# DylanAuty/ObjCAViT

Measured on AMD Instinct MI355X. Metric: images/sec (640x480, bs=16) forward depth inference, 3 batches of 16 in flight per GPU; AbsRel vs CPU ref, higher is better.
Workload: dtype f32 (fp16 / bf16 split contractions)

## Files before the change

include/objcavit_hip.h:

```cpp
#ifndef OBJCAVIT_HIP_H
#define OBJCAVIT_HIP_H

#include <stddef.h>
#include <stdint.h>

#ifdef __cplusplus
extern "C" {
#endif

typedef void* ocv_stream_t;

#define OCV_ABI_VERSION 5
int ocv_abi_version(void);
const char* ocv_last_error(void);

int ocv_range_flag_set(unsigned* flag);
int ocv_range_flag_take_fwd(unsigned* flag, unsigned* out, ocv_stream_t stream);
int ocv_attention_set_fp32_range(int on);
int ocv_attention_set_dispatch(int form);

#define OCV_ACT_NONE 0
#define OCV_ACT_RELU 1
#define OCV_ACT_LEAKY_RELU 2
#define OCV_ACT_SILU 3
// ... 164 lines not shown

int ocv_se_gate_fwd(const float* mean, const float* w1, const float* b1, const float* w2t, const float* b2, float* gate,
                    float* hidden_ws, int B, int C, int R, ocv_stream_t stream);

int ocv_conv_nhwc_fwd(const float* x1, int C1, const float* x2, int C2, const void* w_hi, const void* w_lo,
                      const float* bias, const float* residual, float* y, int B, int H, int W, int Cout, int ksize,
                      int act, ocv_stream_t stream);
int ocv_conv_nhwc_exact_fwd(const float* x1, int C1, const float* x2, int C2, const float* w_tap_major, const float* bias,
                            const float* residual, float* y, int B, int H, int W, int Cout, int ksize, int act,
                            ocv_stream_t stream);
int ocv_conv3x3_nhwc_strided_fwd(const float* x, int Cin, const void* w_hi, const void* w_lo, const float* bias,
                                 const float* residual, float* y, int B, int H, int W, int Cout, int stride, int pad_t,
                                 int pad_l, int Ho, int Wo, int act, ocv_stream_t stream);

int ocv_mbconv_expand_dw_tiles(int Ho, int Wo, int k, int stride);
int ocv_mbconv_expand_dw_fwd(const float* x, const void* w_packed, const float* bias_expand, const float* w_dw,
                             const float* bias_dw, float* y, float* part, int B, int H, int W, int Cin, int mid, int k,
                             int stride, int pad_t, int pad_l, int Ho, int Wo, ocv_stream_t stream);

size_t ocv_split_act_elems(int B, int H, int W, int C);

int ocv_conv_nhwc_split_fwd(const void* x_hl, int Cin, const void* w_hi, const void* w_lo, const float* bias,
                            const float* residual, float* y, void* y_hl, int B, int H, int W, int Cout, int ksize,
                            int act, ocv_stream_t stream);
size_t ocv_conv_nhwc_split_workspace_bytes(int B, int H, int W, int Cin, int Cout, int ksize);
int ocv_conv_nhwc_split_ws_fwd(const void* x_hl, int Cin, const void* w_hi, const void* w_lo, const float* bias,
                               const float* residual, float* y, void* y_hl, int B, int H, int W, int Cout, int ksize,
                               int act, void* workspace, size_t workspace_bytes, ocv_stream_t stream);
int ocv_conv_nhwc_split_x_fwd(const void* x_hl, int Cin, const void* w_hi, const void* w_lo, const float* oscale, int f16,
                              const float* bias, const float* residual, float* y, void* y_hl, int B, int H, int W, int Cout,
                              int ksize, int act, void* workspace, size_t workspace_bytes, ocv_stream_t stream);

int ocv_conv3x3_packed_taps_k(int Cin);
int ocv_conv3x3_split_packed_taps_fwd(const void* x_hl, int Cin, const void* w_hi, const void* w_lo, const float* oscale, int f16,
                                      const float* bias, const float* residual, float* y, void* y_hl, int B, int H, int W, int Cout,
                                      int act, ocv_stream_t stream);

size_t ocv_conv3x3_winograd43_workspace_bytes(int B, int H, int W, int Cin, int Cout);
int ocv_conv3x3_winograd43_split_fwd(const void* x_hl, int Cin, const void* u_hi, const void* u_lo, const float* fscale,
                                     const float* cscale, const float* bias, float* y, void* y_hl, int B, int H, int W, int Cout,
                                     int act, int hl_f16, void* workspace, size_t workspace_bytes, ocv_stream_t stream);

int ocv_tap_interp_supported(int h, int w, int H, int W, int Cout);
int ocv_tap_interp_staging_rounds(int h, int w, int H, int W);
int ocv_tap_interp_combine_fwd(const float* z, int h, int w, int zpad, const float* zborder, const float* s, const float* bias,
                               float* y, void* y_hl, int B, int H, int W, int Cout, int act, ocv_stream_t stream);
int ocv_tap_interp_combine_x_fwd(const float* z, int h, int w, int zpad, const float* zborder, const float* s, const float* bias,
                                 float* y, void* y_hl, int hl_f16, int B, int H, int W, int Cout, int act, ocv_stream_t stream);


int ocv_upsample_concat_split_fwd(const float* x, int h, int w, int C1, const float* skip, int C2, void* out_hl, int B,
                                  int H, int W, ocv_stream_t stream);
int ocv_upsample_concat_split_x_fwd(const float* x, int h, int w, int C1, const float* skip, int C2, void* out_hl, int f16, int B,
                                    int H, int W, ocv_stream_t stream);

size_t ocv_depth_metrics_workspace_bytes(int B, int H, int W);
int ocv_depth_metrics_fwd(const float* pred, const float* pred_mirror, int h, int w, const float* gt, int H, int W,
                          float min_depth, float max_depth, int crop_y0, int crop_y1, int crop_x0, int crop_x1,
                          long first_image_id, float* records, int B, void* workspace, size_t workspace_bytes,
                          ocv_stream_t stream);
size_t ocv_depth_metrics_loss_workspace_bytes(int B, int H, int W, int n_bins);
int ocv_depth_metrics_loss_fwd(const float* pred, const float* pred_mirror, int h, int w, const float* gt, int H, int W,
                               float min_depth, float max_depth, int crop_y0, int crop_y1, int crop_x0, int crop_x1,
                               const float* bin_edges, int n_bins, long first_image_id, float* records, float* loss_records, int B,
                               void* workspace, size_t workspace_bytes, ocv_stream_t stream);

// ... 53 lines not shown
```

objcavit_amd/_lib.py:

```python
from __future__ import annotations

import ctypes as C
import os
from typing import Optional

_HERE = os.path.dirname(os.path.abspath(__file__))
LIB_PATH = os.environ.get("OCV_LIB_PATH") or os.path.join(_HERE, "lib", "libobjcavit_hip.so")

_f32p = C.c_void_p
_u8p = C.c_void_p
_stream = C.c_void_p
ABI_VERSION = 5


class EncoderLayerParams(C.Structure):
    _fields_ = [("struct_size", C.c_size_t)] + [(n, C.c_void_p) for n in (
        "in_proj_w", "in_proj_b", "out_proj_w", "out_proj_b", "norm1_w", "norm1_b",
        "linear1_w", "linear1_b", "linear2_w", "linear2_b", "norm2_w", "norm2_b",
        "in_proj_p3", "out_proj_p3", "linear1_p3", "linear2_p3",
        "in_proj_h2", "out_proj_h2", "linear1_h2", "linear2_h2")]

    def __init__(self, *a, **kw):
        super().__init__(*a, **kw)
        self.struct_size = C.sizeof(EncoderLayerParams)
# ... 106 lines not shown
                                [C.c_int, _f32p, C.c_void_p, C.c_void_p, C.c_void_p, C.c_void_p, C.c_size_t, _stream]),
    "ocv_conv3x3_few_channels_fwd": (C.c_int, [_f32p, C.c_long, C.c_long, C.c_long, C.c_long, _f32p, _f32p] + [C.c_int] * 5 + [_stream]),
    "ocv_stem_conv_fwd": (C.c_int, [_f32p, _f32p, _f32p, _f32p] + [C.c_int] * 12 + [_stream]),
    "ocv_pointwise_packed_weight_elems": (C.c_size_t, [C.c_int, C.c_int]),
    "ocv_pointwise_split_set_dispatch": (C.c_int, [C.c_int, C.c_int, C.c_int]),
    "ocv_pointwise_conv_nhwc_split_fwd": (C.c_int, [_f32p, _f32p, C.c_int, C.c_void_p, _f32p, _f32p, _f32p,
                                                    C.c_long, C.c_int, C.c_int, C.c_int, C.c_void_p]),
    "ocv_pointwise_conv_nhwc_fwd": (C.c_int, [_f32p, _f32p, C.c_int, _f32p, _f32p, _f32p, _f32p, C.c_long, C.c_int, C.c_int,
                                              C.c_int, _stream]),
    "ocv_depthwise_conv_nhwc_fwd": (C.c_int, [_f32p, _f32p, _f32p, _f32p] + [C.c_int] * 11 + [_stream]),
    "ocv_channel_mean_workspace_bytes": (C.c_size_t, [C.c_int, C.c_int, C.c_long]),
    "ocv_channel_mean_nhwc_fwd": (C.c_int, [_f32p, _f32p, C.c_int, C.c_int, C.c_long, C.c_void_p, C.c_size_t, _stream]),
    "ocv_se_gate_fwd": (C.c_int, [_f32p] * 7 + [C.c_int] * 3 + [_stream]),
    "ocv_conv_nhwc_fwd": (C.c_int, [_f32p, C.c_int, _f32p, C.c_int, C.c_void_p, C.c_void_p, _f32p, _f32p, _f32p] +
                          [C.c_int] * 6 + [_stream]),
    "ocv_conv3x3_nhwc_strided_fwd": (C.c_int, [_f32p, C.c_int, C.c_void_p, C.c_void_p, _f32p, _f32p, _f32p] + [C.c_int] * 10 + [_stream]),
    "ocv_conv_nhwc_exact_fwd": (C.c_int, [_f32p, C.c_int, _f32p, C.c_int, _f32p, _f32p, _f32p, _f32p] + [C.c_int] * 6 + [_stream]),
    "ocv_mbconv_expand_dw_tiles": (C.c_int, [C.c_int] * 4),
    "ocv_mbconv_expand_dw_fwd": (C.c_int, [_f32p, C.c_void_p, _f32p, _f32p, _f32p, _f32p, _f32p] + [C.c_int] * 11 + [_stream]),
    "ocv_regressor_bins_fwd": (C.c_int, [_f32p, C.c_long, _f32p, _f32p, _f32p, _f32p, _f32p, _f32p, C.c_int, C.c_int, C.c_int, C.c_int, C.c_float,
                                         C.c_int, C.c_float, C.c_float, _f32p, _f32p, _f32p, C.c_int, _stream]),
    "ocv_bin_edges_fwd": (C.c_int, [_f32p, C.c_int, C.c_float, C.c_float, _f32p, _f32p, _f32p, C.c_int, C.c_int, _stream]),
    "ocv_object_tokens_pad_fwd": (C.c_int, [_f32p, C.c_void_p, C.c_float, _f32p, _u8p, C.c_int, C.c_int, C.c_int, _stream]),
    "ocv_object_front_pad_fwd": (C.c_int, [_f32p, C.c_void_p, C.c_int, C.c_int, C.c_float, _f32p, _u8p] + [C.c_int] * 4 + [_stream]),
    "ocv_split_act_elems": (C.c_size_t, [C.c_int] * 4),
    "ocv_conv_nhwc_split_fwd": (C.c_int, [C.c_void_p, C.c_int, C.c_void_p, C.c_void_p, _f32p, _f32p, _f32p, C.c_void_p]
                                + [C.c_int] * 6 + [_stream]),
    "ocv_conv_nhwc_split_workspace_bytes": (C.c_size_t, [C.c_int] * 6),
    "ocv_conv_nhwc_split_ws_fwd": (C.c_int, [C.c_void_p, C.c_int, C.c_void_p, C.c_void_p, _f32p, _f32p, _f32p, C.c_void_p]
                                   + [C.c_int] * 6 + [C.c_void_p, C.c_size_t, _stream]),
    "ocv_conv_nhwc_split_x_fwd": (C.c_int, [C.c_void_p, C.c_int, C.c_void_p, C.c_void_p, _f32p, C.c_int, _f32p, _f32p, _f32p, C.c_void_p]
                                  + [C.c_int] * 6 + [C.c_void_p, C.c_size_t, _stream]),
    "ocv_conv3x3_packed_taps_k": (C.c_int, [C.c_int]),
    "ocv_conv3x3_split_packed_taps_fwd": (C.c_int, [C.c_void_p, C.c_int, C.c_void_p, C.c_void_p, _f32p, C.c_int, _f32p, _f32p, _f32p, C.c_void_p]
                                          + [C.c_int] * 5 + [_stream]),
    "ocv_upsample_concat_split_x_fwd": (C.c_int, [_f32p, C.c_int, C.c_int, C.c_int, _f32p, C.c_int, C.c_void_p, C.c_int,
                                                  C.c_int, C.c_int, C.c_int, _stream]),
    "ocv_tap_interp_combine_x_fwd": (C.c_int, [_f32p, C.c_int, C.c_int, C.c_int, _f32p, _f32p, _f32p, _f32p, C.c_void_p] + [C.c_int] * 6 + [_stream]),
    "ocv_pos_grid_sample_fwd": (C.c_int, [_f32p, C.c_int, C.c_int, C.c_int, _f32p, C.c_int, C.c_int, C.c_int, C.c_float, C.c_float,
                                          C.c_int, _f32p, _f32p, _stream]),
    "ocv_conv3x3_winograd43_workspace_bytes": (C.c_size_t, [C.c_int] * 5),
    "ocv_conv3x3_winograd43_split_fwd": (C.c_int, [C.c_void_p, C.c_int, C.c_void_p, C.c_void_p, _f32p, _f32p, _f32p, _f32p, C.c_void_p] + [C.c_int] * 6 +
                                         [C.c_void_p, C.c_size_t, _stream]),
    "ocv_tap_interp_supported": (C.c_int, [C.c_int] * 5),
    "ocv_tap_interp_staging_rounds": (C.c_int, [C.c_int] * 4),
    "ocv_tap_interp_combine_fwd": (C.c_int, [_f32p, C.c_int, C.c_int, C.c_int, _f32p, _f32p, _f32p, _f32p, C.c_void_p] + [C.c_int] * 5 + [_stream]),
    "ocv_upsample_concat_split_fwd": (C.c_int, [_f32p, C.c_int, C.c_int, C.c_int, _f32p, C.c_int, C.c_void_p,
                                                C.c_int, C.c_int, C.c_int, _stream]),
}

_lib: Optional[C.CDLL] = None


class HipLibraryError(RuntimeError):
    pass


def load(path: Optional[str] = None) -> C.CDLL:
    global _lib
    if _lib is not None and path is None:
        return _lib
    import torch
    p = path or LIB_PATH
    if not os.path.exists(p):
        raise HipLibraryError(
            f"{p} not found: build it with `python -m objcavit_amd.build` (hipcc --offload-arch=gfx950). "
# ... 24 lines not shown
```

objcavit_amd/csrc/conv_igemm.hip:

```cpp
#include <stdlib.h>

#include "common.hpp"
#include "../../include/objcavit_hip.h"

namespace {

typedef __bf16 bf16x8 __attribute__((ext_vector_type(8)));
typedef _Float16 cv_h16x8 __attribute__((ext_vector_type(8)));
typedef _Float16 cv_h16x4 __attribute__((ext_vector_type(4)));
typedef __bf16 ti4 __attribute__((ext_vector_type(4)));

constexpr int CBM = 256, CBN = 128, CBK = 32;
constexpr int ROWB = 80;
constexpr int A_BYTES = CBM * ROWB, B_BYTES = CBN * ROWB;
constexpr int BUF_BYTES = 2 * A_BYTES + 2 * B_BYTES;

struct ConvArgs {
  const float* x1; const float* x2;
  const __bf16* xhl;
  __bf16* yhl;
  int Cpo;
  const __bf16* whi; const __bf16* wlo;
  const float* bias; const float* res; float* y;
  int C1, C2, Cin, Cp, Cout, H, W, ks, act;
  int Ho, Wo, pad_t, pad_l;
  long M;
  int mtiles, ntiles;
  int ksplit;
  int zbatch;
  long xz_bytes, wz_bytes;
  int zflat;
  int f16;
  const float* oscale;
  unsigned* range_flag;
  unsigned rowpitch;
  int gpt, gpt_inv;
  int Kp;
};

__device__ __forceinline__ f32x4 gload16(const void* p) { return *reinterpret_cast<const f32x4*>(p); }

__device__ __forceinline__ void split4(const f32x4 v, __bf16* hi, __bf16* lo) {
  const float f[4] = {v[0], v[1], v[2], v[3]};
#pragma unroll
  for (int i = 0; i < 4; ++i) {
    const __bf16 h = (__bf16)f[i];
    hi[i] = h;
    lo[i] = (__bf16)(f[i] - (float)h);
  }
}

__device__ __forceinline__ void split4h(const f32x4 v, _Float16* hi, _Float16* lo) {
  const float f[4] = {v[0], v[1], v[2], v[3]};
#pragma unroll
  for (int i = 0; i < 4; ++i) {
    const _Float16 h = (_Float16)f[i];
    hi[i] = h;
    lo[i] = (_Float16)(f[i] - (float)h);
  }
}
template <bool F16>
__device__ __forceinline__ void split4_bits(const f32x4 v, unsigned short* hi, unsigned short* lo) {
  if constexpr (F16) split4h(v, reinterpret_cast<_Float16*>(hi), reinterpret_cast<_Float16*>(lo));
  else split4(v, reinterpret_cast<__bf16*>(hi), reinterpret_cast<__bf16*>(lo));
}
__device__ __forceinline__ void split4_bits(const f32x4 v, unsigned short* hi, unsigned short* lo, bool f16) {
  if (f16) split4_bits<true>(v, hi, lo);
  else split4_bits<false>(v, hi, lo);
}
__device__ __forceinline__ f32x4 join4_bits(const void* p, int lo_off, bool f16) {
// ... 200 lines not shown
  __syncthreads();
  for (int t = 0; t < nsteps; ++t) {
    if ((t & 1) == g) {
      if (t + 2 < nsteps) convert(raw, cvt);
      __syncthreads();
    } else {
      if (t + 1 >= 2 && t + 1 < nsteps) write_lds((t + 1) & 1, raw, cvt);
      if (t + 3 < nsteps) issue_loads(raw);
      __syncthreads();
    }
  }
}

}


namespace {

typedef __attribute__((address_space(1))) const void* gptr_t;
typedef __attribute__((address_space(3))) void* lptr_t;

constexpr int DROW = 64;
constexpr int DA = CBM * DROW, DB = CBN * DROW;
constexpr int DBUF = 2 * DA + 2 * DB;
constexpr int DNBUF = 3;

constexpr int ERS = 68;
__device__ __forceinline__ float conv_act(float v, int act) {
  if (act == OCV_ACT_LEAKY_RELU) return v > 0.f ? v : 0.01f * v;
  if (act == OCV_ACT_SILU) return fast_silu(v);
  if (act == OCV_ACT_RELU) return fmaxf(v, 0.f);
  return v;
}
template <bool F16>
__device__ __forceinline__ void conv_store_rows(const ConvArgs& p, const unsigned char* lds, int wave, int lane, long m0, int n0,
                                                long yoff) {
  const int cw = wave & 3, half = wave >> 2;
  const int wm = cw >> 1, wn = cw & 1;
  const float* tile = reinterpret_cast<const float*>(lds) + cw * (128 * ERS);
  const int oct = lane & 7, rsub = lane >> 3;
  const int ncol = n0 + wn * 64 + oct * 8;
  if (ncol >= p.Cout) return;
  float bv[8], sv[8];
#pragma unroll
  for (int e = 0; e < 8; ++e) {
    bv[e] = p.bias != nullptr ? p.bias[ncol + e] : 0.f;
    sv[e] = p.oscale != nullptr ? p.oscale[ncol + e] : 1.f;
  }
  float amax = 0.f;
#pragma unroll 4
  for (int it = 0; it < 8; ++it) {
    const int row = half * 64 + it * 8 + rsub;
    const long m = m0 + wm * 128 + row;
    if (m >= p.M) continue;
    f32x4 a = *reinterpret_cast<const f32x4*>(tile + row * ERS + oct * 8);
    f32x4 c = *reinterpret_cast<const f32x4*>(tile + row * ERS + oct * 8 + 4);
#pragma unroll
    for (int e = 0; e < 4; ++e) {
      a[e] = conv_act(fmaf(a[e], sv[e], bv[e]), p.act);
      c[e] = conv_act(fmaf(c[e], sv[4 + e], bv[4 + e]), p.act);
    }
    const long o = m * p.Cout + ncol;
    if (p.res != nullptr) {
      a += *reinterpret_cast<const f32x4*>(p.res + o);
      c += *reinterpret_cast<const f32x4*>(p.res + o + 4);
    }
    if (p.y != nullptr) {
      *reinterpret_cast<f32x4*>(p.y + yoff + o) = a;
      *reinterpret_cast<f32x4*>(p.y + yoff + o + 4) = c;
    }
    if (p.yhl != nullptr) {
      __attribute__((aligned(16))) unsigned short hi[8], lo[8];
      split4_bits<F16>(a, hi, lo);
      split4_bits<F16>(c, hi + 4, lo + 4);
      if constexpr (F16) amax = ocv_amax4(ocv_amax4(amax, a), c);
      const long oh = hl_index(m, ncol, p.Cpo);
      *reinterpret_cast<bf16x8*>(p.yhl + oh) = *reinterpret_cast<bf16x8*>(hi);
      *reinterpret_cast<bf16x8*>(p.yhl + oh + 32) = *reinterpret_cast<bf16x8*>(lo);
    }
  }
  if constexpr (F16) ocv_range_note(p.range_flag, amax);
}

template <bool F16>
__global__ __launch_bounds__(512) void conv_split_dma_kernel(ConvArgs p) {
  extern __shared__ __attribute__((aligned(1024))) unsigned char lds[];
// ... 54 lines not shown
        bl[j] = *reinterpret_cast<const bf16x8*>(pb + DB + j * 16 * DROW);
      }
#pragma unroll
      for (int i = 0; i < 8; ++i) {
        ah[i] = *reinterpret_cast<const bf16x8*>(pa + i * 16 * DROW);
        al[i] = *reinterpret_cast<const bf16x8*>(pa + DA + i * 16 * DROW);
      }
#pragma unroll
      for (int i = 0; i < 8; ++i)
#pragma unroll
        for (int j = 0; j < 4; ++j) {
          if constexpr (F16) {
            acc[i][j] = __builtin_amdgcn_mfma_f32_16x16x32_f16(__builtin_bit_cast(cv_h16x8, ah[i]), __builtin_bit_cast(cv_h16x8, bh[j]), acc[i][j], 0, 0, 0);
            acc[i][j] = __builtin_amdgcn_mfma_f32_16x16x32_f16(__builtin_bit_cast(cv_h16x8, ah[i]), __builtin_bit_cast(cv_h16x8, bl[j]), acc[i][j], 0, 0, 0);
            acc[i][j] = __builtin_amdgcn_mfma_f32_16x16x32_f16(__builtin_bit_cast(cv_h16x8, al[i]), __builtin_bit_cast(cv_h16x8, bh[j]), acc[i][j], 0, 0, 0);
          } else {
            acc[i][j] = __builtin_amdgcn_mfma_f32_16x16x32_bf16(ah[i], bh[j], acc[i][j], 0, 0, 0);
            acc[i][j] = __builtin_amdgcn_mfma_f32_16x16x32_bf16(ah[i], bl[j], acc[i][j], 0, 0, 0);
            acc[i][j] = __builtin_amdgcn_mfma_f32_16x16x32_bf16(al[i], bh[j], acc[i][j], 0, 0, 0);
          }
        }
      __syncthreads();
    }

    if ((p.Cout & 7) == 0) {
      float* tile = reinterpret_cast<float*>(lds) + wave * (128 * ERS);
#pragma unroll
      for (int j = 0; j < 4; ++j)
#pragma unroll
        for (int i = 0; i < 8; ++i)
#pragma unroll
          for (int r = 0; r < 4; ++r) tile[(16 * i + 4 * q4 + r) * ERS + 16 * j + l15] = acc[i][j][r];
      __syncthreads();
      conv_store_rows<F16>(p, lds, wave, lane, m0, n0, yoff);
      return;
    }
#pragma unroll
    for (int j = 0; j < 4; ++j) {
      const int n = n0 + wn * 64 + j * 16 + l15;
      const bool nok = n < p.Cout;
      const float bv = (p.bias != nullptr && nok) ? p.bias[n] : 0.f;
      const float sv = (p.oscale != nullptr && nok) ? p.oscale[n] : 1.f;
#pragma unroll
      for (int i = 0; i < 8; ++i)
#pragma unroll
        for (int r = 0; r < 4; ++r) {
          const long m = m0 + wm * 128 + i * 16 + 4 * q4 + r;
          if (nok && m < p.M) {
            float v = fmaf(acc[i][j][r], sv, bv);
            if (p.act == OCV_ACT_LEAKY_RELU) v = v > 0.f ? v : 0.01f * v;
            else if (p.act == OCV_ACT_SILU) v = fast_silu(v);
            else if (p.act == OCV_ACT_RELU) v = fmaxf(v, 0.f);
            if (p.res != nullptr) v += p.res[m * p.Cout + n];
            if (p.y != nullptr) p.y[yoff + m * p.Cout + n] = v;
            if (p.yhl != nullptr) {
              if constexpr (F16) {
                ocv_range_note(p.range_flag, fabsf(v));
                _Float16* yh = reinterpret_cast<_Float16*>(p.yhl);
                const _Float16 hb = (_Float16)v;
                yh[hl_index(m, n, p.Cpo)] = hb;
                yh[hl_index(m, n, p.Cpo) + 32] = (_Float16)(v - (float)hb);
              } else {
                const __bf16 hb = (__bf16)v;
                p.yhl[hl_index(m, n, p.Cpo)] = hb;
                p.yhl[hl_index(m, n, p.Cpo) + 32] = (__bf16)(v - (float)hb);
              }
            }
// ... 94 lines not shown
    for (int i = 0; i < 2; ++i) {
      unsigned char* dst = base + 2 * DA + (32 * pw + 16 * i) * DROW;
      __builtin_amdgcn_global_load_lds((gptr_t)(whz_ + woff + rbB[i]), (lptr_t)dst, 16, 0, 0);
      __builtin_amdgcn_global_load_lds((gptr_t)(wlz_ + woff + rbB[i]), (lptr_t)(dst + DB), 16, 0, 0);
    }
  };

  auto issue_dma = [&](int buf) {
    if (p.gpt > 0) issue_dma_packed(buf);
    else issue_dma_dense(buf);
  };

#define OCV_WAIT_VM(N) asm volatile("s_waitcnt vmcnt(" #N ")" ::: "memory")
  issue_dma(0);
  if (nsteps > 1) {
    issue_dma(1);
    OCV_WAIT_VM(12);
  } else {
    OCV_WAIT_VM(0);
  }
  __builtin_amdgcn_s_barrier();
  for (int t = 0; t < nsteps; ++t) {
    if (t + 2 < nsteps) {
      issue_dma((t + 2) % DNBUF);
      OCV_WAIT_VM(12);
    } else {
      OCV_WAIT_VM(0);
    }
    __builtin_amdgcn_s_barrier();
  }
#undef OCV_WAIT_VM
  if ((p.Cout & 7) == 0) {
    __syncthreads();
    conv_store_rows<F16>(p, lds, wave, lane, m0, n0, yoff);
  }
}


struct FinArgs {
  const float *part, *bias, *res;
  float* y;
  __bf16* yhl;
  long M, items;
  int Cout, Cpo, act, ksplit;
  const float* oscale;
  int f16;
  unsigned* range_flag;
};

__global__ __launch_bounds__(256) void conv_splitk_finish_kernel(FinArgs p) {
  const long i = (long)blockIdx.x * 256 + threadIdx.x;
  if (i >= p.items) return;
  const int noct = p.Cout >> 3;
  const long m = i / noct;
  const int n = (int)(i - m * noct) * 8;
  const long o = m * p.Cout + n;
  f32x4 a = *reinterpret_cast<const f32x4*>(p.part + o), c = *reinterpret_cast<const f32x4*>(p.part + o + 4);
  for (int k = 1; k < p.ksplit; ++k) {
    a += *reinterpret_cast<const f32x4*>(p.part + k * p.M * p.Cout + o);
    c += *reinterpret_cast<const f32x4*>(p.part + k * p.M * p.Cout + o + 4);
  }
#pragma unroll
  for (int e = 0; e < 4; ++e) {
    a[e] = conv_act(fmaf(a[e], p.oscale != nullptr ? p.oscale[n + e] : 1.f, p.bias != nullptr ? p.bias[n + e] : 0.f), p.act);
    c[e] = conv_act(fmaf(c[e], p.oscale != nullptr ? p.oscale[n + 4 + e] : 1.f, p.bias != nullptr ? p.bias[n + 4 + e] : 0.f), p.act);
  }
  if (p.res != nullptr) {
    a += *reinterpret_cast<const f32x4*>(p.res + o);
    c += *reinterpret_cast<const f32x4*>(p.res + o + 4);
  }
  if (p.y != nullptr) {
    *reinterpret_cast<f32x4*>(p.y + o) = a;
    *reinterpret_cast<f32x4*>(p.y + o + 4) = c;
  }
  if (p.yhl != nullptr) {
    __attribute__((aligned(16))) unsigned short hi[8], lo[8];
    split4_bits(a, hi, lo, p.f16 != 0);
    split4_bits(c, hi + 4, lo + 4, p.f16 != 0);
    if (p.f16 != 0) ocv_range_note(p.range_flag, ocv_amax4(ocv_amax4(0.f, a), c));
    const long oh = hl_index(m, n, p.Cpo);
    *reinterpret_cast<bf16x8*>(p.yhl + oh) = *reinterpret_cast<bf16x8*>(hi);
    *reinterpret_cast<bf16x8*>(p.yhl + oh + 32) = *reinterpret_cast<bf16x8*>(lo);
  }
}

}

namespace {
int conv_ksplit(long M, int Cout, int Cin, int ksize) {
  const long tiles = (long)ocv_cdiv(M, CBM) * ocv_cdiv(Cout, CBN);
  const int nsteps = ksize * ksize * ((Cin + CBK - 1) / CBK);
  if ((Cout & 7) != 0 || nsteps < 128 || tiles <= 256) return 1;
  const double c1 = (double)((tiles + 255) / 256), c2 = (double)((2 * tiles + 255) / 256) / 2.0;
  return c2 <= 0.9 * c1 ? 2 : 1;
}
int launch_conv(ConvArgs& a, int B, hipStream_t st) {
  a.Cp = (a.Cin + CBK - 1) / CBK * CBK;
  a.M = (long)B * a.H * a.W;
  a.mtiles = ocv_cdiv(a.M, CBM); a.ntiles = ocv_cdiv(a.Cout, CBN);
  static bool attr = false;
  if (!attr) {
    (void)hipFuncSetAttribute((const void*)conv_split_dma_kernel<false>, hipFuncAttributeMaxDynamicSharedMemorySize, 160 * 1024);
    (void)hipFuncSetAttribute((const void*)conv_split_dma_kernel<true>, hipFuncAttributeMaxDynamicSharedMemorySize, 160 * 1024);
    attr = true;
  }
  if (a.ksplit < 1) a.ksplit = 1;
  if (a.zbatch < 1) a.zbatch = 1;
  const unsigned parts = a.zflat > 0 ? a.zflat : a.ksplit * a.zbatch;
  if (a.f16)
    hipLaunchKernelGGL(conv_split_dma_kernel<true>, dim3(a.mtiles * a.ntiles * parts), dim3(512), DNBUF * DBUF, st, a);
  else
    hipLaunchKernelGGL(conv_split_dma_kernel<false>, dim3(a.mtiles * a.ntiles * parts), dim3(512), DNBUF * DBUF, st, a);
  OCV_CHECK_LAUNCH("ocv_conv_nhwc");
  return 0;
}

template <int KS, int S, bool CAT>
int launch_igemm(ConvArgs& a, int B, hipStream_t st, const char* name) {
  a.Cp = (a.Cin + CBK - 1) / CBK * CBK;
  a.M = (long)B * a.Ho * a.Wo;
  a.mtiles = ocv_cdiv(a.M, CBM); a.ntiles = ocv_cdiv(a.Cout, CBN);
  static bool attr = false;
  if (!attr) {
    (void)hipFuncSetAttribute((const void*)conv_igemm_kernel<KS, S, CAT>, hipFuncAttributeMaxDynamicSharedMemorySize, 160 * 1024);
    attr = true;
  }
  hipLaunchKernelGGL((conv_igemm_kernel<KS, S, CAT>), dim3(a.mtiles * a.ntiles), dim3(512), 2 * BUF_BYTES, st, a);
  OCV_CHECK_LAUNCH(name);
  return 0;
}
}

extern "C" size_t ocv_split_act_elems(int B, int H, int W, int C) {
  if (B < 1 || H < 1 || W < 1 || C < 1) return 0;
  return (size_t)B * H * W * 2 * ((C + 31) / 32 * 32);
}

extern "C" size_t ocv_conv_nhwc_split_workspace_bytes(int B, int H, int W, int Cin, int Cout, int ksize) {
  if (B < 1 || H < 1 || W < 1 || Cin < 1 || Cout < 1 || (ksize != 1 && ksize != 3)) return 0;
  const long M = (long)B * H * W;
  const int ks = conv_ksplit(M, Cout, Cin, ksize);
  return ks > 1 ? (size_t)ks * M * Cout * sizeof(float) : 0;
}

extern "C" int ocv_conv_nhwc_split_x_fwd(const void* x_hl, int Cin, const void* w_hi, const void* w_lo, const float* oscale,
                                         int f16, const float* bias, const float* residual, float* y, void* y_hl, int B, int H,
                                         int W, int Cout, int ksize, int act, void* workspace, size_t workspace_bytes,
                                         ocv_stream_t stream) {
  OCV_CHECK_ARG(x_hl && w_hi && w_lo && (y || y_hl), "ocv_conv_nhwc_split_fwd: null pointer");
  OCV_CHECK_ARG(ocv_aligned16(y) && ocv_aligned16(y_hl) && ocv_aligned16(residual) && ocv_aligned16(workspace), "ocv_conv_nhwc_split_fwd: outputs, residual and workspace must be 16-byte aligned");
  OCV_CHECK_ARG(ksize == 1 || ksize == 3, "ocv_conv_nhwc_split_fwd: kernel size must be 1 or 3 (got %d)", ksize);
  OCV_CHECK_ARG(B >= 1 && H >= 1 && W >= 1 && Cout >= 1 && Cin >= 1, "ocv_conv_nhwc_split_fwd: bad sizes");
  OCV_CHECK_ARG(act >= 0 && act <= 3, "ocv_conv_nhwc_split_fwd: unknown activation %d", act);
  OCV_CHECK_ARG((reinterpret_cast<uintptr_t>(x_hl) & 127) == 0 && ocv_aligned16(w_hi) && ocv_aligned16(w_lo), "ocv_conv_nhwc_split_fwd: x_hl must be 128-byte aligned, weights 16-byte aligned");
  OCV_CHECK_ARG((long)B * H * W * (Cin + 32) * 4 < (1L << 32) && 9L * Cout * (Cin + 32) * 2 < (1L << 32), "ocv_conv_nhwc_split_fwd: each operand must be smaller than 4 GiB");
  OCV_CHECK_ARG(f16 == 0 || f16 == 1, "ocv_conv_nhwc_split_fwd: f16 must be 0 (bf16 pairs) or 1 (fp16 pairs)");
  ConvArgs a{};
  a.xhl = (const __bf16*)x_hl; a.yhl = (__bf16*)y_hl; a.Cpo = (Cout + 31) / 32 * 32;
  a.whi = (const __bf16*)w_hi; a.wlo = (const __bf16*)w_lo; a.bias = bias; a.res = residual; a.y = y;
  a.C1 = Cin; a.C2 = 0; a.Cin = Cin; a.Cout = Cout; a.H = H; a.W = W; a.ks = ksize; a.act = act; a.ksplit = 1;
  a.f16 = f16; a.oscale = oscale;
  a.range_flag = (f16 && y_hl != nullptr) ? ocv_range_flag_current() : nullptr;
  if (y_hl != nullptr && Cout % 32 != 0) {
    const int zrc = ocv_zero_async(y_hl, ocv_split_act_elems(B, H, W, Cout) * sizeof(__bf16), (hipStream_t)stream);
    if (zrc != 0) return zrc;
  }
  const long M = (long)B * H * W;
  const int ks = conv_ksplit(M, Cout, Cin, ksize);
  if (ks > 1 && workspace != nullptr && workspace_bytes >= (size_t)ks * M * Cout * sizeof(float)) {
    ConvArgs h = a;
    h.bias = nullptr; h.res = nullptr; h.yhl = nullptr; h.act = OCV_ACT_NONE; h.y = (float*)workspace; h.ksplit = ks; h.oscale = nullptr;
    const int rc = launch_conv(h, B, (hipStream_t)stream);
    if (rc != 0) return rc;
    FinArgs f{(const float*)workspace, bias, residual, y, (__bf16*)y_hl, M, M * Cout / 8, Cout, a.Cpo, act, ks, oscale, f16, a.range_flag};
    hipLaunchKernelGGL(conv_splitk_finish_kernel, dim3((unsigned)((f.items + 255) / 256)), dim3(256), 0, (hipStream_t)stream, f);
    OCV_CHECK_LAUNCH("ocv_conv_nhwc_split_fwd(finish)");
    return 0;
  }
  return launch_conv(a, B, (hipStream_t)stream);
}

extern "C" int ocv_conv3x3_packed_taps_k(int Cin) {
  if (Cin < 1 || Cin > 2040) return 0;
  const int gpt = (Cin + 7) / 8;
  return (9 * gpt + 3) / 4 * CBK;
}

extern "C" int ocv_conv3x3_split_packed_taps_fwd(const void* x_hl, int Cin, const void* w_hi, const void* w_lo, const float* oscale,
                                                 int f16, const float* bias, const float* residual, float* y, void* y_hl, int B,
                                                 int H, int W, int Cout, int act, ocv_stream_t stream) {
  OCV_CHECK_ARG(x_hl && w_hi && w_lo && (y || y_hl), "ocv_conv3x3_split_packed_taps_fwd: null pointer");
  OCV_CHECK_ARG(ocv_aligned16(y) && ocv_aligned16(y_hl) && ocv_aligned16(residual), "ocv_conv3x3_split_packed_taps_fwd: outputs and residual must be 16-byte aligned");
  OCV_CHECK_ARG(B >= 1 && H >= 1 && W >= 1 && Cout >= 1 && Cin >= 8 && Cin % 8 == 0 && Cin <= 2040,
                "ocv_conv3x3_split_packed_taps_fwd: bad sizes (Cin must be a multiple of 8 in [8, 2040], got %d)", Cin);
  OCV_CHECK_ARG(act >= 0 && act <= 3, "ocv_conv3x3_split_packed_taps_fwd: unknown activation %d", act);
  OCV_CHECK_ARG(f16 == 0 || f16 == 1, "ocv_conv3x3_split_packed_taps_fwd: f16 must be 0 (bf16 pairs) or 1 (fp16 pairs)");
  OCV_CHECK_ARG((reinterpret_cast<uintptr_t>(x_hl) & 127) == 0 && ocv_aligned16(w_hi) && ocv_aligned16(w_lo),
                "ocv_conv3x3_split_packed_taps_fwd: x_hl must be 128-byte aligned, weights 16-byte aligned");
// ... 468 lines not shown
```

Before: 1108.

## Add halo-staged 3x3 conv kernel reusing input tile across taps

Adds a new 3x3 implicit-GEMM conv kernel that stages an 8x32 spatial tile plus halo of the split hi/lo input into LDS once per channel chunk and reuses it for all nine taps. Weights for each tap stream through a small ring buffer, and the input is double-buffered by dedicated producer waves. The goal is to remove the repeated per-tap global loads of input rows made by the existing tap-ring kernel. Auto-dispatch enables it only for two specific shapes (240x320x128 and 120x160x256); other shapes keep the old path. The cost is extra LDS use and a larger, more complex kernel.

```diff
diff --git a/include/objcavit_hip.h b/include/objcavit_hip.h
--- a/include/objcavit_hip.h
+++ b/include/objcavit_hip.h
@@ -220,6 +220,10 @@
                               int ksize, int act, void* workspace, size_t workspace_bytes, ocv_stream_t stream);
 
 int ocv_conv3x3_packed_taps_k(int Cin);
+int ocv_conv3x3_halo_supported(int B, int H, int W, int Cin, int Cout);
+size_t ocv_conv3x3_halo_lds_bytes(void);
+int ocv_conv3x3_set_dispatch(int mode);
+int ocv_conv3x3_last_kernel(void);
 int ocv_conv3x3_split_packed_taps_fwd(const void* x_hl, int Cin, const void* w_hi, const void* w_lo, const float* oscale, int f16,
                                       const float* bias, const float* residual, float* y, void* y_hl, int B, int H, int W, int Cout,
                                       int act, ocv_stream_t stream);
diff --git a/objcavit_amd/_lib.py b/objcavit_amd/_lib.py
--- a/objcavit_amd/_lib.py
+++ b/objcavit_amd/_lib.py
@@ -162,6 +162,10 @@
     "ocv_conv_nhwc_split_x_fwd": (C.c_int, [C.c_void_p, C.c_int, C.c_void_p, C.c_void_p, _f32p, C.c_int, _f32p, _f32p, _f32p, C.c_void_p]
                                   + [C.c_int] * 6 + [C.c_void_p, C.c_size_t, _stream]),
     "ocv_conv3x3_packed_taps_k": (C.c_int, [C.c_int]),
+    "ocv_conv3x3_halo_supported": (C.c_int, [C.c_int] * 5),
+    "ocv_conv3x3_halo_lds_bytes": (C.c_size_t, []),
+    "ocv_conv3x3_set_dispatch": (C.c_int, [C.c_int]),
+    "ocv_conv3x3_last_kernel": (C.c_int, []),
     "ocv_conv3x3_split_packed_taps_fwd": (C.c_int, [C.c_void_p, C.c_int, C.c_void_p, C.c_void_p, _f32p, C.c_int, _f32p, _f32p, _f32p, C.c_void_p]
                                           + [C.c_int] * 5 + [_stream]),
     "ocv_upsample_concat_split_x_fwd": (C.c_int, [_f32p, C.c_int, C.c_int, C.c_int, _f32p, C.c_int, C.c_void_p, C.c_int,
diff --git a/objcavit_amd/csrc/conv_igemm.hip b/objcavit_amd/csrc/conv_igemm.hip
--- a/objcavit_amd/csrc/conv_igemm.hip
+++ b/objcavit_amd/csrc/conv_igemm.hip
@@ -1,4 +1,6 @@
 #include <stdlib.h>
+
+#include <type_traits>
 
 #include "common.hpp"
 #include "../../include/objcavit_hip.h"
@@ -36,6 +38,7 @@
   unsigned rowpitch;
   int gpt, gpt_inv;
   int Kp;
+  int halo;
 };
 
 __device__ __forceinline__ f32x4 gload16(const void* p) { return *reinterpret_cast<const f32x4*>(p); }
@@ -302,8 +305,8 @@
   if (act == OCV_ACT_RELU) return fmaxf(v, 0.f);
   return v;
 }
-template <bool F16>
-__device__ __forceinline__ void conv_store_rows(const ConvArgs& p, const unsigned char* lds, int wave, int lane, long m0, int n0,
+template <bool F16, class RowMap>
+__device__ __forceinline__ void conv_store_rows(const ConvArgs& p, const unsigned char* lds, int wave, int lane, RowMap rowm, int n0,
                                                 long yoff) {
   const int cw = wave & 3, half = wave >> 2;
   const int wm = cw >> 1, wn = cw & 1;
@@ -321,7 +324,7 @@
 #pragma unroll 4
   for (int it = 0; it < 8; ++it) {
     const int row = half * 64 + it * 8 + rsub;
-    const long m = m0 + wm * 128 + row;
+    const long m = rowm(wm * 128 + row);
     if (m >= p.M) continue;
     f32x4 a = *reinterpret_cast<const f32x4*>(tile + row * ERS + oct * 8);
     f32x4 c = *reinterpret_cast<const f32x4*>(tile + row * ERS + oct * 8 + 4);
@@ -442,7 +445,7 @@
 #pragma unroll
           for (int r = 0; r < 4; ++r) tile[(16 * i + 4 * q4 + r) * ERS + 16 * j + l15] = acc[i][j][r];
       __syncthreads();
-      conv_store_rows<F16>(p, lds, wave, lane, m0, n0, yoff);
+      conv_store_rows<F16>(p, lds, wave, lane, [m0](int R) { return m0 + R; }, n0, yoff);
       return;
     }
 #pragma unroll
@@ -603,7 +606,228 @@
 #undef OCV_WAIT_VM
   if ((p.Cout & 7) == 0) {
     __syncthreads();
-    conv_store_rows<F16>(p, lds, wave, lane, m0, n0, yoff);
+    conv_store_rows<F16>(p, lds, wave, lane, [m0](int R) { return m0 + R; }, n0, yoff);
+  }
+}
+
+constexpr int HTY = 8, HTX = 32, HPITCH = 40;
+constexpr int HROWS = (HTY + 2) * HPITCH;
+constexpr int HPLANE = HROWS * DROW, HABUF = 2 * HPLANE;
+constexpr int HPIECES = 2 * HROWS / 16;
+constexpr int HAPW = (HPIECES + 3) / 4;
+constexpr int HW0 = 2 * HABUF, HWSLOT = 2 * DB;
+constexpr int HLDS = HW0 + DNBUF * HWSLOT;
+static_assert(HROWS % 16 == 0 && HLDS <= 160 * 1024 && 4 * 128 * ERS * 4 <= HLDS, "conv_halo_dma_kernel: LDS budget");
+__host__ __device__ constexpr int halo_na(int T) { return T < 5 ? 2 : (T < 8 ? 1 : 0); }
+__host__ __device__ constexpr int halo_a0(int T) { return T < 5 ? 2 * T : 5 + T; }
+static_assert(halo_a0(8) == HAPW && halo_a0(7) + halo_na(7) == HAPW, "conv_halo_dma_kernel: A pieces per chunk");
+
+template <int N>
+__device__ __forceinline__ void halo_wait_vm() { asm volatile("s_waitcnt vmcnt(%0)" ::"n"(N) : "memory"); }
+
+template <bool F16>
+__global__ __launch_bounds__(512) void conv_halo_dma_kernel(ConvArgs p) {
+  extern __shared__ __attribute__((aligned(1024))) unsigned char lds[];
+
+  const int tid = threadIdx.x, lane = tid & 63, wave = tid >> 6;
+  int wg = blockIdx.x;
+  {
+    const int nwg = p.mtiles * p.ntiles;
+    const int q = nwg >> 3, r = nwg & 7, xcd = wg & 7, idx = wg >> 3;
+    wg = (xcd < r ? xcd * (q + 1) : r * (q + 1) + (xcd - r) * q) + idx;
+  }
+  const int nchunk = p.Cp / CBK, nsteps = 9 * nchunk;
+  const int mt = wg / p.ntiles, nt = wg - mt * p.ntiles;
+  const int n0 = nt * CBN;
+  const int ppr = p.W / HTX, ppi = (p.H / HTY) * ppr;
+  const int img = mt / ppi, prem = mt - img * ppi;
+  const int ty0 = (prem / ppr) * HTY, tx0 = (prem % ppr) * HTX;
+  const long mbase = ((long)img * p.H + ty0) * p.W + tx0;
+  const int Wd = p.W;
+  auto rowm = [mbase, Wd](int R) { return mbase + (long)(R >> 5) * Wd + (R & 31); };
+
+  if (wave < 4) {
+    const int wm = wave >> 1, wn = wave & 1;
+    const int l15 = lane & 15, q4 = lane >> 4;
+    unsigned aofs[3];
+#pragma unroll
+    for (int kx = 0; kx < 3; ++kx)
+      aofs[kx] = (unsigned)(((wm * 4) * HPITCH + l15 + kx) * DROW + ((q4 ^ (((l15 + kx) >> 1) & 3)) * 16));
+    const unsigned char* pbw = lds + HW0 + (wn * 64 + l15) * DROW + ((q4 ^ ((l15 >> 1) & 3)) * 16);
+    f32x4 acc[8][4];
+#pragma unroll
+    for (int i = 0; i < 8; ++i)
+#pragma unroll
+      for (int j = 0; j < 4; ++j) acc[i][j] = f32x4{0.f, 0.f, 0.f, 0.f};
+
+    __syncthreads();
+    for (int c = 0; c < nchunk; ++c) {
+      const unsigned char* abuf = lds + (c & 1) * HABUF;
+#pragma unroll 1
+      for (int ky = 0; ky < 3; ++ky) {
+#pragma unroll
+        for (int kx = 0; kx < 3; ++kx) {
+          const unsigned char* pa = abuf + ky * (HPITCH * DROW) + aofs[kx];
+          const unsigned char* pb = pbw + kx * HWSLOT;
+          bf16x8 ah[8], al[8], bh[4], bl[4];
+#pragma unroll
+          for (int j = 0; j < 4; ++j) {
+            bh[j] = *reinterpret_cast<const bf16x8*>(pb + j * 16 * DROW);
+            bl[j] = *reinterpret_cast<const bf16x8*>(pb + DB + j * 16 * DROW);
+          }
+#pragma unroll
+          for (int i = 0; i < 8; ++i) {
+            ah[i] = *reinterpret_cast<const bf16x8*>(pa + ((i >> 1) * HPITCH + (i & 1) * 16) * DROW);
+            al[i] = *reinterpret_cast<const bf16x8*>(pa + HPLANE + ((i >> 1) * HPITCH + (i & 1) * 16) * DROW);
+          }
+#pragma unroll
+          for (int i = 0; i < 8; ++i)
+#pragma unroll
+            for (int j = 0; j < 4; ++j) {
+              if constexpr (F16) {
+                acc[i][j] = __builtin_amdgcn_mfma_f32_16x16x32_f16(__builtin_bit_cast(cv_h16x8, ah[i]), __builtin_bit_cast(cv_h16x8, bh[j]), acc[i][j], 0, 0, 0);
+                acc[i][j] = __builtin_amdgcn_mfma_f32_16x16x32_f16(__builtin_bit_cast(cv_h16x8, ah[i]), __builtin_bit_cast(cv_h16x8, bl[j]), acc[i][j], 0, 0, 0);
+                acc[i][j] = __builtin_amdgcn_mfma_f32_16x16x32_f16(__builtin_bit_cast(cv_h16x8, al[i]), __builtin_bit_cast(cv_h16x8, bh[j]), acc[i][j], 0, 0, 0);
+              } else {
+                acc[i][j] = __builtin_amdgcn_mfma_f32_16x16x32_bf16(ah[i], bh[j], acc[i][j], 0, 0, 0);
+                acc[i][j] = __builtin_amdgcn_mfma_f32_16x16x32_bf16(ah[i], bl[j], acc[i][j], 0, 0, 0);
+                acc[i][j] = __builtin_amdgcn_mfma_f32_16x16x32_bf16(al[i], bh[j], acc[i][j], 0, 0, 0);
+              }
+            }
+          __syncthreads();
+        }
+      }
+    }
+
+    if ((p.Cout & 7) == 0) {
+      float* tile = reinterpret_cast<float*>(lds) + wave * (128 * ERS);
+#pragma unroll
+      for (int j = 0; j < 4; ++j)
+#pragma unroll
+        for (int i = 0; i < 8; ++i)
+#pragma unroll
+          for (int r = 0; r < 4; ++r) tile[(16 * i + 4 * q4 + r) * ERS + 16 * j + l15] = acc[i][j][r];
+      __syncthreads();
+      conv_store_rows<F16>(p, lds, wave, lane, rowm, n0, 0L);
+      return;
+    }
+    const long mlane = mbase + (long)(wm * 4) * Wd + 4 * q4;
+#pragma unroll
+    for (int j = 0; j < 4; ++j) {
+      const int n = n0 + wn * 64 + j * 16 + l15;
+      const bool nok = n < p.Cout;
+      const float bv = (p.bias != nullptr && nok) ? p.bias[n] : 0.f;
+      const float sv = (p.oscale != nullptr && nok) ? p.oscale[n] : 1.f;
+#pragma unroll
+      for (int i = 0; i < 8; ++i)
+#pragma unroll
+        for (int r = 0; r < 4; ++r) {
+          const long m = mlane + (i >> 1) * Wd + ((i & 1) * 16 + r);
+          if (nok) {
+            float v = fmaf(acc[i][j][r], sv, bv);
+            if (p.act == OCV_ACT_LEAKY_RELU) v = v > 0.f ? v : 0.01f * v;
+            else if (p.act == OCV_ACT_SILU) v = fast_silu(v);
+            else if (p.act == OCV_ACT_RELU) v = fmaxf(v, 0.f);
+            if (p.res != nullptr) v += p.res[m * p.Cout + n];
+            if (p.y != nullptr) p.y[m * p.Cout + n] = v;
+            if (p.yhl != nullptr) {
+              if constexpr (F16) {
+                ocv_range_note(p.range_flag, fabsf(v));
+                _Float16* yh = reinterpret_cast<_Float16*>(p.yhl);
+                const _Float16 hb = (_Float16)v;
+                yh[hl_index(m, n, p.Cpo)] = hb;
+                yh[hl_index(m, n, p.Cpo) + 32] = (_Float16)(v - (float)hb);
+              } else {
+                const __bf16 hb = (__bf16)v;
+                p.yhl[hl_index(m, n, p.Cpo)] = hb;
+                p.yhl[hl_index(m, n, p.Cpo) + 32] = (__bf16)(v - (float)hb);
+              }
+            }
+          }
+        }
+    }
+    return;
+  }
+
+  const int pw = wave - 4;
+  const int lrow = lane >> 2;
+  const int lchunk = (lane & 3) ^ ((lane >> 3) & 3);
+  unsigned aoff[HAPW], amask = 0, adst[HAPW];
+#pragma unroll
+  for (int j = 0; j < HAPW; ++j) {
+    const int q = min(4 * j + pw, HPIECES - 1);
+    const int plane = q & 1, pc = q >> 1;
+    const int hp = pc * 16 + lrow, hy = hp / HPITCH, hx = hp - hy * HPITCH;
+    const int y = ty0 - 1 + hy, x = tx0 - 1 + hx;
+    const bool ok = hx < HTX + 2 && (unsigned)y < (unsigned)p.H && (unsigned)x < (unsigned)p.W;
+    aoff[j] = (((unsigned)img * (unsigned)p.H + (unsigned)y) * (unsigned)p.W + (unsigned)x) * (unsigned)(4 * p.Cp) +
+              (unsigned)(plane * 64 + lchunk * 16);
+    amask |= ok ? 1u << j : 0u;
+    adst[j] = (unsigned)(plane * HPLANE + pc * 1024);
+  }
+  unsigned rbB[2];
+#pragma unroll
+  for (int i = 0; i < 2; ++i) {
+    const int bn = min(n0 + 32 * pw + 16 * i + lrow, p.Cout - 1);
+    rbB[i] = (unsigned)(((long)bn * p.Cp + lchunk * 8) * 2);
+  }
+  const unsigned wtap = (unsigned)((long)p.Cout * p.Cp * 2);
+  const char* xz = (const char*)p.xhl;
+  const char* whz = (const char*)p.whi;
+  const char* wlz = (const char*)p.wlo;
+
+  auto issue_a = [&](int j, int c) {
+    const void* src = ((amask >> j) & 1u) ? (const void*)(xz + aoff[j] + (unsigned)c * 128u) : (const void*)ocv_zero_page;
+    __builtin_amdgcn_global_load_lds((gptr_t)src, (lptr_t)(lds + (c & 1) * HABUF + adst[j]), 16, 0, 0);
+  };
+  auto issue_w = [&](int tap, int c) {
+    const unsigned woff = (unsigned)tap * wtap + (unsigned)c * (CBK * 2);
+    unsigned char* base = lds + HW0 + (tap % 3) * HWSLOT;
+#pragma unroll
+    for (int i = 0; i < 2; ++i) {
+      unsigned char* dst = base + (32 * pw + 16 * i) * DROW;
+      __builtin_amdgcn_global_load_lds((gptr_t)(whz + woff + rbB[i]), (lptr_t)dst, 16, 0, 0);
+      __builtin_amdgcn_global_load_lds((gptr_t)(wlz + woff + rbB[i]), (lptr_t)(dst + DB), 16, 0, 0);
+    }
+  };
+
+  auto step = [&](auto tc, int c) {
+    constexpr int T = decltype(tc)::value;
+    const bool nxt = c + 1 < nchunk;
+    if (nxt) {
+#pragma unroll
+      for (int k = 0; k < halo_na(T); ++k) issue_a(halo_a0(T) + k, c + 1);
+    }
+    if (9 * c + T + 2 < nsteps) {
+      issue_w((T + 2) % 9, c + (T + 2) / 9);
+      if (nxt) halo_wait_vm<4 + halo_na(T)>();
+      else halo_wait_vm<4>();
+    } else {
+      halo_wait_vm<0>();
+    }
+    __builtin_amdgcn_s_barrier();
+  };
+
+#pragma unroll
+  for (int j = 0; j < HAPW; ++j) issue_a(j, 0);
+  issue_w(0, 0);
+  issue_w(1, 0);
+  halo_wait_vm<4>();
+  __builtin_amdgcn_s_barrier();
+  for (int c = 0; c < nchunk; ++c) {
+    step(std::integral_constant<int, 0>{}, c);
+    step(std::integral_constant<int, 1>{}, c);
+    step(std::integral_constant<int, 2>{}, c);
+    step(std::integral_constant<int, 3>{}, c);
+    step(std::integral_constant<int, 4>{}, c);
+    step(std::integral_constant<int, 5>{}, c);
+    step(std::integral_constant<int, 6>{}, c);
+    step(std::integral_constant<int, 7>{}, c);
+    step(std::integral_constant<int, 8>{}, c);
+  }
+  if ((p.Cout & 7) == 0) {
+    __syncthreads();
+    conv_store_rows<F16>(p, lds, wave, lane, rowm, n0, 0L);
   }
 }
 
@@ -658,13 +882,24 @@
 }
 
 namespace {
+constexpr int KSPLIT_MIN_STEPS = 128;
 int conv_ksplit(long M, int Cout, int Cin, int ksize) {
   const long tiles = (long)ocv_cdiv(M, CBM) * ocv_cdiv(Cout, CBN);
   const int nsteps = ksize * ksize * ((Cin + CBK - 1) / CBK);
-  if ((Cout & 7) != 0 || nsteps < 128 || tiles <= 256) return 1;
+  if ((Cout & 7) != 0 || nsteps < KSPLIT_MIN_STEPS || tiles <= 256) return 1;
   const double c1 = (double)((tiles + 255) / 256), c2 = (double)((2 * tiles + 255) / 256) / 2.0;
   return c2 <= 0.9 * c1 ? 2 : 1;
 }
+int g_conv3x3_dispatch = 0;
+
+bool conv_halo_auto(int , int H, int W, int Cin, int Cout) {
+  static const int won[][4] = {{240, 320, 128, 128}, {120, 160, 256, 256}};
+  for (const auto& s : won)
+    if (H == s[0] && W == s[1] && Cin == s[2] && Cout == s[3]) return true;
+  return false;
+}
+int g_conv3x3_last_kernel = 0;
+
 int launch_conv(ConvArgs& a, int B, hipStream_t st) {
   a.Cp = (a.Cin + CBK - 1) / CBK * CBK;
   a.M = (long)B * a.H * a.W;
@@ -673,7 +908,18 @@
   if (!attr) {
     (void)hipFuncSetAttribute((const void*)conv_split_dma_kernel<false>, hipFuncAttributeMaxDynamicSharedMemorySize, 160 * 1024);
     (void)hipFuncSetAttribute((const void*)conv_split_dma_kernel<true>, hipFuncAttributeMaxDynamicSharedMemorySize, 160 * 1024);
+    (void)hipFuncSetAttribute((const void*)conv_halo_dma_kernel<false>, hipFuncAttributeMaxDynamicSharedMemorySize, 160 * 1024);
+    (void)hipFuncSetAttribute((const void*)conv_halo_dma_kernel<true>, hipFuncAttributeMaxDynamicSharedMemorySize, 160 * 1024);
     attr = true;
+  }
+  if (a.ks == 3 && a.gpt == 0) g_conv3x3_last_kernel = a.halo ? 2 : 1;
+  if (a.halo) {
+    if (a.f16)
+      hipLaunchKernelGGL(conv_halo_dma_kernel<true>, dim3(a.mtiles * a.ntiles), dim3(512), HLDS, st, a);
+    else
+      hipLaunchKernelGGL(conv_halo_dma_kernel<false>, dim3(a.mtiles * a.ntiles), dim3(512), HLDS, st, a);
+    OCV_CHECK_LAUNCH("ocv_conv_nhwc");
+    return 0;
   }
   if (a.ksplit < 1) a.ksplit = 1;
   if (a.zbatch < 1) a.zbatch = 1;
@@ -712,6 +958,23 @@
   const long M = (long)B * H * W;
   const int ks = conv_ksplit(M, Cout, Cin, ksize);
   return ks > 1 ? (size_t)ks * M * Cout * sizeof(float) : 0;
+}
+
+extern "C" int ocv_conv3x3_halo_supported(int B, int H, int W, int Cin, int Cout) {
+  if (B < 1 || H < 1 || W < 1 || Cin < 1 || Cout < 1) return 0;
+  if (H % HTY != 0 || W % HTX != 0 || 9 * ((Cin + CBK - 1) / CBK) >= KSPLIT_MIN_STEPS) return 0;
+  if ((long)B * H * W * (Cin + 32) * 4 >= (1L << 32) || 9L * Cout * (Cin + 32) * 2 >= (1L << 32)) return 0;
+  return 1;
+}
+
+extern "C" size_t ocv_conv3x3_halo_lds_bytes(void) { return (size_t)HLDS; }
+
+extern "C" int ocv_conv3x3_last_kernel(void) { return g_conv3x3_last_kernel; }
+
+extern "C" int ocv_conv3x3_set_dispatch(int mode) {
+  OCV_CHECK_ARG(mode >= 0 && mode <= 2, "ocv_conv3x3_set_dispatch: mode must be 0 (automatic), 1 (tap ring) or 2 (halo-staged), got %d", mode);
+  g_conv3x3_dispatch = mode;
+  return 0;
 }
 
 extern "C" int ocv_conv_nhwc_split_x_fwd(const void* x_hl, int Cin, const void* w_hi, const void* w_lo, const float* oscale,
@@ -726,6 +989,12 @@
   OCV_CHECK_ARG((reinterpret_cast<uintptr_t>(x_hl) & 127) == 0 && ocv_aligned16(w_hi) && ocv_aligned16(w_lo), "ocv_conv_nhwc_split_fwd: x_hl must be 128-byte aligned, weights 16-byte aligned");
   OCV_CHECK_ARG((long)B * H * W * (Cin + 32) * 4 < (1L << 32) && 9L * Cout * (Cin + 32) * 2 < (1L << 32), "ocv_conv_nhwc_split_fwd: each operand must be smaller than 4 GiB");
   OCV_CHECK_ARG(f16 == 0 || f16 == 1, "ocv_conv_nhwc_split_fwd: f16 must be 0 (bf16 pairs) or 1 (fp16 pairs)");
+  bool use_halo = false;
+  if (ksize == 3 && g_conv3x3_dispatch != 1) {
+    const bool can = ocv_conv3x3_halo_supported(B, H, W, Cin, Cout) != 0;
+    OCV_CHECK_ARG(can || g_conv3x3_dispatch != 2, "ocv_conv_nhwc_split_fwd: the halo-staged 3x3 kernel is forced (ocv_conv3x3_set_dispatch(2)) and cannot run B %d, %d x %d, %d -> %d channels (ocv_conv3x3_halo_supported: H %% 8 == 0, W %% 32 == 0, fewer than %d K steps)", B, H, W, Cin, Cout, KSPLIT_MIN_STEPS);
+    use_halo = can && (g_conv3x3_dispatch == 2 || conv_halo_auto(B, H, W, Cin, Cout));
+  }
   ConvArgs a{};
   a.xhl = (const __bf16*)x_hl; a.yhl = (__bf16*)y_hl; a.Cpo = (Cout + 31) / 32 * 32;
   a.whi = (const __bf16*)w_hi; a.wlo = (const __bf16*)w_lo; a.bias = bias; a.res = residual; a.y = y;
@@ -735,6 +1004,10 @@
   if (y_hl != nullptr && Cout % 32 != 0) {
     const int zrc = ocv_zero_async(y_hl, ocv_split_act_elems(B, H, W, Cout) * sizeof(__bf16), (hipStream_t)stream);
     if (zrc != 0) return zrc;
+  }
+  if (use_halo) {
+    a.halo = 1;
+    return launch_conv(a, B, (hipStream_t)stream);
   }
   const long M = (long)B * H * W;
   const int ks = conv_ksplit(M, Cout, Cin, ksize);
```

After: 1129 (median of 6 runs). 1.02x the previous value.
